# jkulhanek/tetra-nerf

Hardware: NVIDIA H100
Metric: rays/sec (4096-ray batch, 300k-tet mesh) (higher is better)
Workload: dtype f32 (trace/interp/compositing) + f16w2 tensor-core MLP (fp16 activations x fp16 hi/lo weights, f32 accumulate; per-sample density/colour within 1e-4 of the fp32 oracle, tests/test_gpu_render.py)

## Files before the change

### tetra-nerf_b200/csrc/tn_common.cuh

```cuda
#pragma once
#include <cuda_runtime.h>
#include <stdint.h>

#include <atomic>
#include <string>

#include "../../include/tetranerf_b200.h"

#define TN_EMPTY 0xFFFFFFFFu

namespace tn {

void set_error(const std::string &msg);
int fail(int code, const std::string &msg);

#define TN_CUDA(expr)                                                                                       \
    do {                                                                                                    \
        cudaError_t _e = (expr);                                                                            \
        if (_e != cudaSuccess)                                                                              \
            return tn::fail(TN_ERR_CUDA, std::string(#expr) + " failed: " + cudaGetErrorString(_e) + " (" + \
                                             __FILE__ + ":" + std::to_string(__LINE__) + ")");              \
    } while (0)

#define TN_TRY(...)                              \
    do {                                         \
        const int _rc = (__VA_ARGS__);           \
        if (_rc != TN_OK) return _rc;            \
    } while (0)

inline std::atomic<uint64_t> g_device_bytes{0};

template <typename T>
struct DevArray {
    T *p = nullptr;
    size_t cap = 0;

    DevArray() = default;
    DevArray(const DevArray &) = delete;
    DevArray &operator=(const DevArray &) = delete;
    DevArray(DevArray &&o) noexcept : p(o.p), cap(o.cap) { o.p = nullptr; o.cap = 0; }
    DevArray &operator=(DevArray &&o) noexcept {
        if (this != &o) {
            release();
            p = o.p; cap = o.cap;
            o.p = nullptr; o.cap = 0;
        }
        return *this;
    }
    ~DevArray() { release(); }

    int grow(size_t n) {
        if (n <= cap) return TN_OK;
        release();
        const size_t bytes = (n * sizeof(T) + 255) / 256 * 256;
        void *q = nullptr;
        TN_CUDA(cudaMalloc(&q, bytes));
        p = static_cast<T *>(q);
        cap = bytes / sizeof(T);
        g_device_bytes += cap * sizeof(T);
        return TN_OK;
    }

// ... 300 lines not shown
```

### tetra-nerf_b200/csrc/tn_render.cu

```cuda
#include <atomic>
#include <cmath>
#include <vector>

#include <cstddef>
#include <cstdlib>
#include <cub/cub.cuh>
#include "tn_background.cuh"
#include "tn_common.cuh"
#include "tn_composite.cuh"
#include "tn_direnc.cuh"
#include "tn_mlp.cuh"
#include "tn_mlp_bwd.cuh"
#include "tn_mlp_pack.cuh"
#include "tn_sort.cuh"

namespace tn {

int launch_trace_internal(tn_tracer *h, const float *o, const float *d, uint32_t R, uint32_t M, uint32_t *num, uint32_t *cells, float *bary,
                          float *dist, uint32_t *verts, int dense, cudaStream_t s);

struct TrainBufs {
    uint32_t *n_active;
    uint32_t *ray_list;
    float *ebins_f, *sbins_f;
    uint4 *vi_f;
    float *bary_f;
    float *out_f;
    float *dirbias, *enc;
    float *dirs;
};

constexpr uint32_t SAVED_MAGIC = 0x53564e54u;
struct SavedHeader {
    uint32_t magic, R, M, Sc, Sf, S2, det;
    uint32_t edepth;
    float bg[3];
    uint32_t pad2;
    uint64_t gen;
    uint64_t mesh_gen;
    uint32_t cull;
    uint32_t live_c, live_f;
    uint32_t pad3;
    uint32_t bgmap;
    uint32_t bg_H, bg_W, pad4;
    uint64_t bg_gen;
};

struct RenderState {
    DevArray<float> fshadow;
    uint32_t V = 0;
    DevArray<uint8_t> wimg;
    DevArray<uint8_t> wimg16;
    int mlp_prec = 2;
    DevArray<float> bias;
    DevArray<float> head;
    DevArray<float> w4dir;
    bool have_weights = false;
    uint64_t gen = 0;
    DevArray<uint32_t> num, cells, verts;
    DevArray<float> bary, dist;
    DevArray<float> ebins_c, sbins_c, bary_c, dens_c;
    DevArray<uint4> vi_c;
    DevArray<uint8_t> own;
    TrainBufs own_b{};
    SavedHeader last{};
    DevArray<uint8_t> wimg_bwd;
    DevArray<float4> dout;
    DevArray<float> gshadow, gw, g_dirbias;
    float *peer[8] = {nullptr, nullptr, nullptr, nullptr, nullptr, nullptr, nullptr, nullptr};
    uint32_t gather_world = 0, gather_rank = 0, gather_stride = 0;
    bool profile = false;
    cudaEvent_t ev[7] = {nullptr, nullptr, nullptr, nullptr, nullptr, nullptr, nullptr};
// ... 73 lines not shown
    const uint32_t v0 = blockIdx.x * 32;
    for (uint32_t c = threadIdx.y; c < 64; c += blockDim.y) {
        const uint32_t v = v0 + threadIdx.x;
        tile[c][threadIdx.x] = v < V ? in[(size_t)c * V + v] : 0.f;
    }
    __syncthreads();
    for (uint32_t r = threadIdx.y; r < 32; r += blockDim.y) {
        const uint32_t v = v0 + r;
        if (v < V) {
            out[(size_t)v * 64 + field_pos(threadIdx.x)] = tile[threadIdx.x][r];
            out[(size_t)v * 64 + field_pos(32 + threadIdx.x)] = tile[32 + threadIdx.x][r];
        }
    }
}

__global__ void k_pack_small(const float *b1, const float *b2, const float *b3, const float *w4, const float *b4, const float *wc,
                             const float *bc, const float *wd, const float *bd, float *bias, float *head, float *w4dir) {
    const int t = threadIdx.x;
    bias[t] = b1[t]; bias[128 + t] = b2[t]; bias[256 + t] = b3[t];
    head[t] = wd[t];
    head[128 + t] = wc[t]; head[256 + t] = wc[128 + t]; head[384 + t] = wc[256 + t];
    if (t == 0) { head[512] = bd[0]; head[513] = bc[0]; head[514] = bc[1]; head[515] = bc[2]; }
    for (int k = 0; k < 27; ++k) w4dir[t * 27 + k] = w4[t * 155 + k];
    w4dir[128 * 27 + t] = b4[t];
}

constexpr int SAMPLE_WARPS = 4;

struct SampleParams {
    uint32_t R, M, Sc, Sf, S2, biased;
    const uint32_t *num;
    const float2 *dist;
    const uint4 *verts;
    const float *bary;
    const float *o, *d;
    uint32_t *n_active, *ray_list;
    float *ebins_c, *sbins_c, *bary_c;
    uint4 *vi_c;
    const float *dens_c;
    float *ebins_f, *bary_f;
    uint4 *vi_f;
    float *dirbias;
    const float *w4dir;
    const float *out_f;
    float *rgb, *acc, *depth;
    uint8_t *mask;
    float far_plane, bg0, bg1, bg2;
    uint32_t train;
    const float *jit_c, *jit_f;
    float *sbins_f, *enc;
    float *peer[8];
    uint32_t gather_world, gather_rank, gather_stride;
    const uint32_t *ray_slot;
    float *edepth;
    uint32_t *dbounds;
    const uint32_t *cells;
    const float *occ;
    float occ_thr;
    const float *bgmap;
    uint32_t bg_H, bg_W;
};

#define TN_CULLED 0xFFFFFFFEu
__device__ __forceinline__ bool cell_culled(const SampleParams &p, uint32_t cell) { return cell != TN_EMPTY && __ldg(p.occ + cell) < p.occ_thr; }
__device__ __forceinline__ void cull_sample(const SampleParams &p, size_t row, uint32_t seg, uint4 &vi, float &b0, float &b1, float &b2) {
    if (vi.x == TN_EMPTY) return;
    if (cell_culled(p, __ldg(p.cells + row + seg))) {
        vi = make_uint4(TN_EMPTY, TN_EMPTY, TN_EMPTY, TN_CULLED);
        b0 = b1 = b2 = 0.f;
    }
}

__device__ __forceinline__ void store_pixel(const SampleParams &p, uint32_t ray, int lane, float r, float g, float b, float a, float depth, uint8_t mask) {
    if (lane == 0) {
        p.rgb[3 * (size_t)ray] = r; p.rgb[3 * (size_t)ray + 1] = g; p.rgb[3 * (size_t)ray + 2] = b;
        p.acc[ray] = a; p.depth[ray] = depth;
        if (p.mask != nullptr) p.mask[ray] = mask;
    }
    if ((uint32_t)lane < p.gather_world) {
        float2 *dst = reinterpret_cast<float2 *>(p.peer[lane] + 6 * ((size_t)p.gather_rank * p.gather_stride + ray));
        dst[0] = make_float2(r, g); dst[1] = make_float2(b, a); dst[2] = make_float2(depth, mask ? 1.f : 0.f);
        __threadfence_system();
    }
}

__device__ void smem_scan_max(const float *in, float *out, uint32_t n, int lane) {
    float carry = -3.0e38f;
    for (uint32_t base = 0; base < n; base += 32) {
        const uint32_t i = base + lane;
        float v = i < n ? in[i] : -3.0e38f;
#pragma unroll
        for (int o = 1; o < 32; o <<= 1) {
            const float t = __shfl_up_sync(0xffffffffu, v, o);
            if (lane >= o) v = fmaxf(v, t);
        }
        v = fmaxf(v, carry);
        if (i < n) out[i] = v;
        carry = __shfl_sync(0xffffffffu, v, 31);
    }
    __syncwarp();
}
__device__ __forceinline__ float linspace_f(float start, float end, uint32_t steps, uint32_t i) {
    const float step = (end - start) / (float)(steps - 1);
    return i < steps / 2 ? start + step * (float)i : end - step * (float)(steps - i - 1);
}

__device__ __forceinline__ uint32_t match_sample(float d, uint32_t n, const float2 *__restrict__ dist, const float *pm, size_t row,
                                                 const uint4 *__restrict__ verts, const float *__restrict__ bary, uint4 &vi, float &b0,
                                                 float &b1, float &b2) {
    vi = make_uint4(TN_EMPTY, TN_EMPTY, TN_EMPTY, TN_EMPTY);
    b0 = b1 = b2 = 0.f;
    uint32_t lo = 0, hi = n;
    while (lo < hi) {
        const uint32_t mid = (lo + hi) >> 1;
        if (pm[mid] < d) lo = mid + 1; else hi = mid;
    }
    if (lo >= n) return lo;
    const float2 h = __ldg(dist + row + lo);
    if (h.x <= d) {
        vi = __ldg(verts + row + lo);
        const float mult = __fdiv_rn(__fsub_rn(d, h.x), __fsub_rn(h.y, h.x));
        const float omm = __fsub_rn(1.0f, mult);
        const float *c = bary + 6 * (row + lo);
        b0 = __fadd_rn(__fmul_rn(omm, __ldg(c)), __fmul_rn(mult, __ldg(c + 3)));
        b1 = __fadd_rn(__fmul_rn(omm, __ldg(c + 1)), __fmul_rn(mult, __ldg(c + 4)));
        b2 = __fadd_rn(__fmul_rn(omm, __ldg(c + 2)), __fmul_rn(mult, __ldg(c + 5)));
    }
    return lo;
}

__host__ __device__ __forceinline__ size_t seg_arr(uint32_t M) { return (size_t)M + 2; }
__host__ __device__ __forceinline__ size_t coarse_floats(uint32_t M, uint32_t Sc, uint32_t biased) { return seg_arr(M) * (biased ? 2 : 1) + (size_t)Sc + 2; }
__host__ __device__ __forceinline__ size_t fine_floats(uint32_t M, uint32_t Smax) { return seg_arr(M) + 4 * ((size_t)Smax + 2); }
__host__ __device__ __forceinline__ size_t place_floats(uint32_t M, uint32_t Sc) { return 3 * seg_arr(M) + (size_t)Sc + 2; }

template <bool ORDERED, bool PLACE = false>
__global__ void __launch_bounds__(SAMPLE_WARPS * 32) k_sample_coarse(const SampleParams p) {
    extern __shared__ float sm[];
    const int warp = threadIdx.x >> 5, lane = threadIdx.x & 31;
    const uint32_t ray = blockIdx.x * SAMPLE_WARPS + warp;
    if (ray >= p.R) return;
    const uint32_t M = p.M, S = p.Sc;
    const size_t A = seg_arr(M);
    float *pm = sm + (size_t)warp * (PLACE ? place_floats(M, S) : coarse_floats(M, S, p.biased));
    float *cum = pm + A, *e = PLACE ? cum + 2 * A : cum + (p.biased ? A : 0);
    const uint32_t n = p.num[ray];
    if constexpr (ORDERED) {
        if (ray == p.R - 1 && lane == 0) *p.n_active = p.ray_slot[ray] + (n > 0 ? 1u : 0u);
    }
    if (n == 0) {
        float b0 = p.bg0, b1 = p.bg1, b2 = p.bg2;
        if (p.bgmap != nullptr) {
            bg_lookup(p.bgmap, p.bg_H, p.bg_W, p.d[3 * (size_t)ray], p.d[3 * (size_t)ray + 1], p.d[3 * (size_t)ray + 2], b0, b1, b2);
            if (!p.train) { b0 = fminf(fmaxf(b0, 0.f), 1.f); b1 = fminf(fmaxf(b1, 0.f), 1.f); b2 = fminf(fmaxf(b2, 0.f), 1.f); }
        }
        store_pixel(p, ray, lane, b0, b1, b2, 0.f, p.far_plane, 0);
        return;
    }
    uint32_t slot = 0;
    if constexpr (ORDERED) {
        slot = p.ray_slot[ray];
        if (lane == 0) { p.ray_list[slot] = ray; p.mask[ray] = 1; }
    } else {
        if (lane == 0) { slot = atomicAdd(p.n_active, 1u); p.ray_list[slot] = ray; p.mask[ray] = 1; }
        slot = __shfl_sync(0xffffffffu, slot, 0);
    }
    const size_t row = (size_t)ray * M;
    const float near = __ldg(&p.dist[row]).x, far = __ldg(&p.dist[row + n - 1]).y;
    bool placed = false;
    uint32_t nk = 0;
    uint32_t *kix = reinterpret_cast<uint32_t *>(cum + A);
    if constexpr (PLACE) {
        for (uint32_t base = 0; base < n; base += 32) {
            const uint32_t k = base + lane;
            const bool kept = k < n && !cell_culled(p, __ldg(p.cells + row + k));
            const uint32_t bal = __ballot_sync(0xffffffffu, kept);
            if (kept) kix[nk + __popc(bal & ((1u << lane) - 1u))] = k;
            nk += __popc(bal);
        }
        placed = nk > 0 && nk < n;
    }
    for (uint32_t k = lane; k < n; k += 32) {
        const float2 h = __ldg(&p.dist[row + k]);
        pm[k] = h.y;
        if (p.biased && !placed) cum[k + 1] = fmaxf(h.y - h.x, 0.f);
    }
    if (p.biased && !placed && lane == 0) cum[0] = near;
    if (placed && !p.biased) {
        __syncwarp();
        for (uint32_t i = lane; i < nk; i += 32) {
            const float2 h = __ldg(&p.dist[row + kix[i]]);
            cum[i + 1] = fmaxf(h.y - h.x, 0.f);
        }
        if (lane == 0) cum[0] = 0.f;
    }
    __syncwarp();
    smem_scan_max(pm, pm, n, lane);
    if (p.biased && !placed) {
        smem_scan_add(cum, n + 1, lane);
    }
    if (placed) {
        if (!p.biased) smem_scan_add(cum, nk + 1, lane);
        for (uint32_t j = lane; j <= S; j += 32) {
            float b = linspace_f(0.f, 1.f, S + 1, j);
            if (p.jit_c != nullptr) {
                const float lower = j == 0 ? b : (b + linspace_f(0.f, 1.f, S + 1, j - 1)) / 2.0f;
                const float upper = j == S ? b : (linspace_f(0.f, 1.f, S + 1, j + 1) + b) / 2.0f;
                b = lower + (upper - lower) * __ldg(p.jit_c + (size_t)ray * (S + 1) + j);
            }
// ... 11 lines not shown
            } else {
                const float x = b * cum[nk];
                uint32_t lo = 1, hi = nk;
                while (lo < hi) { const uint32_t mid = (lo + hi) >> 1; if (cum[mid] <= x) lo = mid + 1; else hi = mid; }
                i = lo - 1;
                off = x - cum[i];
            }
            const float2 h = __ldg(&p.dist[row + kix[i]]);
            e[j] = fminf(h.x + off, fmaxf(h.x, h.y));
        }
        __syncwarp();
        smem_scan_max(e, e, S + 1, lane);
        for (uint32_t j = lane; j <= S; j += 32) {
            p.ebins_c[(size_t)slot * (S + 1) + j] = e[j];
            p.sbins_c[(size_t)slot * (S + 1) + j] = (e[j] - near) / (far - near);
        }
    } else {
        for (uint32_t j = lane; j <= S; j += 32) {
            float b = linspace_f(0.f, 1.f, S + 1, j);
            if (p.jit_c != nullptr) {
                const float lower = j == 0 ? b : (b + linspace_f(0.f, 1.f, S + 1, j - 1)) / 2.0f;
                const float upper = j == S ? b : (linspace_f(0.f, 1.f, S + 1, j + 1) + b) / 2.0f;
                b = lower + (upper - lower) * __ldg(p.jit_c + (size_t)ray * (S + 1) + j);
            }
            float eu = b * far + (1.f - b) * near;
            float sb = b;
            if (p.biased) {
                const float uni = (eu - near) / (far - near);
                float rest = uni * (float)n;
                float iv = fminf(floorf(rest), (float)(n - 1));
                iv = fmaxf(iv, 0.f);
                rest = rest - iv;
                const uint32_t k = (uint32_t)iv;
                const float2 hk = __ldg(&p.dist[row + k]);
                const float len = fmaxf(hk.y - hk.x, 0.f);
                eu = cum[k] + len * rest;
                sb = (eu - near) / (far - near);
            }
            e[j] = eu;
            p.ebins_c[(size_t)slot * (S + 1) + j] = eu;
            p.sbins_c[(size_t)slot * (S + 1) + j] = sb;
        }
    }
    __syncwarp();
    for (uint32_t j = lane; j < S; j += 32) {
        const float dmid = (e[j + 1] + e[j]) / 2.f;
        uint4 vi; float b0, b1, b2;
        const uint32_t seg = match_sample(dmid, n, p.dist, pm, row, p.verts, p.bary, vi, b0, b1, b2);
        if (p.occ != nullptr) cull_sample(p, row, seg, vi, b0, b1, b2);
        const size_t g = (size_t)slot * S + j;
        p.vi_c[g] = vi;
        p.bary_c[3 * g] = b0; p.bary_c[3 * g + 1] = b1; p.bary_c[3 * g + 2] = b2;
    }
}

__device__ __forceinline__ void dir_bias(const SampleParams &p, uint32_t ray, uint32_t slot, int lane) {
    const float dx = p.d[3 * (size_t)ray], dy = p.d[3 * (size_t)ray + 1], dz = p.d[3 * (size_t)ray + 2];
    float enc[27];
    encode_direction(dx, dy, dz, enc);
    if (p.train) {
#pragma unroll
        for (int k = 0; k < 27; ++k) if (lane == k) p.enc[(size_t)slot * 27 + k] = enc[k];
    }
    for (uint32_t o = lane; o < 128; o += 32) {
        float acc = p.w4dir[128 * 27 + o];
#pragma unroll
        for (int k = 0; k < 27; ++k) acc = fmaf(__ldg(p.w4dir + o * 27 + k), enc[k], acc);
        p.dirbias[(size_t)slot * 128 + o] = acc;
    }
}

__global__ void __launch_bounds__(SAMPLE_WARPS * 32) k_sample_fine(const SampleParams p) {
    extern __shared__ float sm[];
    const int warp = threadIdx.x >> 5, lane = threadIdx.x & 31;
    const uint32_t slot = blockIdx.x * SAMPLE_WARPS + warp;
    if (slot >= *p.n_active) return;
    const uint32_t M = p.M, S = p.Sc, S2 = p.S2, nb = p.Sf + 1;
    const size_t A = seg_arr(M), B = (size_t)max(p.Sc, p.S2) + 2;
    float *pm = sm + (size_t)warp * fine_floats(M, max(p.Sc, p.S2));
    float *cdf = pm + A, *e = cdf + B, *x = e + B, *y = x + B;
    const uint32_t ray = p.ray_list[slot];
    const uint32_t n = p.num[ray];
    const size_t row = (size_t)ray * M;
    const float near = __ldg(&p.dist[row]).x, far = __ldg(&p.dist[row + n - 1]).y;
    for (uint32_t k = lane; k < n; k += 32) pm[k] = __ldg(&p.dist[row + k]).y;
    __syncwarp();
    smem_scan_max(pm, pm, n, lane);
    const float *eb = p.ebins_c + (size_t)slot * (S + 1);
    const float *sbc = p.sbins_c + (size_t)slot * (S + 1);
    for (uint32_t j = lane; j < S; j += 32) x[j] = (eb[j + 1] - eb[j]) * p.dens_c[(size_t)slot * S + j];
    __syncwarp();
    weights_from_density(x, y, S, lane);
    float part = 0.f;
    for (uint32_t j = lane; j < S; j += 32) { x[j] = x[j] + 0.01f; part += x[j]; }
    float wsum = warp_sum_f(part);
    const float padding = fmaxf(1e-5f - wsum, 0.f);
    wsum += padding;
    for (uint32_t j = lane; j < S; j += 32) y[j] = (x[j] + padding / (float)S) / wsum;
    __syncwarp();
    smem_scan_add(y, S, lane);
    if (lane == 0) cdf[0] = 0.f;
    for (uint32_t j = lane; j < S; j += 32) cdf[j + 1] = fminf(1.f, y[j]);
    __syncwarp();
    const float u_end = (float)(1.0 - 1.0 / (double)nb), u_off = (float)(1.0 / (2.0 * (double)nb));
    for (uint32_t i = lane; i < nb; i += 32) {
        const float u = linspace_f(0.f, u_end, nb, i) + (p.jit_f != nullptr ? __ldg(p.jit_f + (size_t)ray * nb + i) / (float)nb : u_off);
// ... 606 lines not shown
    if (r && r->gather_world && d_normals != nullptr)
        return fail(TN_ERR_ARG, "tn_render: the fused pixel gather (tn_render_set_gather) carries no normals; switch it off first");
    if (!r || !r->fshadow.p || !r->have_weights) return fail(TN_ERR_STATE, "tn_render: call tn_render_set_field and tn_render_set_weights first");
    if (!h->mesh.nodes.p) return fail(TN_ERR_STATE, "tn_render: no tetrahedra loaded");
    if (r->V != h->mesh.V) return fail(TN_ERR_ARG, "tn_render: field has a different vertex count than the mesh");
    const uint32_t M = cfg->max_ray_triangles, Sc = cfg->num_samples, Sf = cfg->num_fine_samples;
    if (Sc == 0 || Sc > 4096 || Sf > 4096) return fail(TN_ERR_ARG, "tn_render: num_samples must be in [1,4096]");
    if (tf != nullptr && Sf == 0) return fail(TN_ERR_ARG, "tn_render_train_forward: the fused training step needs num_fine_samples > 0");
    const bool det = tf != nullptr && r->det;
    if (det && (uint64_t)R * (Sc + Sf + 1) * 4 > 0x7FFFFFFFull)
        return fail(TN_ERR_ARG, "tn_render_train_forward: deterministic mode takes at most 2^29 fine samples per call (split the batch)");
    if (R == 0) return TN_OK;
    if ((uint64_t)R * (uint64_t)(Sc + Sf + 1) >= (1ull << 32)) return fail(TN_ERR_ARG, "tn_render: rays x samples must stay below 2^32 per call (split the batch)");
    const bool single = Sf == 0;
    const bool cull = r->occ != nullptr;
    if (cull && r->occ_T != h->mesh.T)
        return fail(TN_ERR_STATE, "tn_render: the occupancy was set for a mesh with another number of tetrahedra (tn_render_set_occupancy)");
    const uint32_t S2 = single ? Sc : Sc + Sf + 1;
    DeviceGuard g(h->device);
    cudaStream_t s = (cudaStream_t)stream;
    const bool place = cull && r->occ_place;
    const size_t smem_sc = SAMPLE_WARPS * sizeof(float) * (place ? place_floats(M, Sc) : coarse_floats(M, Sc, cfg->use_biased_sampler));
    const size_t smem_sf = SAMPLE_WARPS * sizeof(float) * fine_floats(M, std::max(Sc, S2));
    const size_t smem_c = SAMPLE_WARPS * sizeof(float) * 2 * ((size_t)S2 + 2);
    const size_t smem_cb = SAMPLE_WARPS * sizeof(float) * 4 * ((size_t)S2 + 2);
    if (!r->smem_optin) TN_CUDA(cudaDeviceGetAttribute(&r->smem_optin, cudaDevAttrMaxSharedMemoryPerBlockOptin, h->device));
    {
        size_t need = std::max(smem_sc, smem_c);
        const char *kern = smem_sc >= smem_c ? "k_sample_coarse" : "k_composite";
        if (!single && smem_sf > need) { need = smem_sf; kern = "k_sample_fine"; }
        if (tf != nullptr && smem_cb > need) { need = smem_cb; kern = "k_composite_bwd"; }
        if (need > (size_t)r->smem_optin)
            return fail(TN_ERR_ARG, "tn_render: num_samples + num_fine_samples = " + std::to_string(Sc + Sf) + " at max_ray_triangles = " +
                                        std::to_string(M) + " needs " + std::to_string(need) + " bytes of shared memory per block in " + kern +
                                        ", above the device's shared-memory limit of " + std::to_string(r->smem_optin) +
                                        " bytes (fewer samples or a smaller max_ray_triangles)");
    }
    TN_TRY(ensure_ws(r, R, M, Sc));
    const bool own = tf == nullptr || tf->saved == nullptr;
    const bool keep_dirs = tf != nullptr && r->bgmap != nullptr;
    if (own) TN_TRY(r->own.grow(saved_layout(R, S2, nullptr, nullptr, tf == nullptr, keep_dirs)));
    if (d_normals != nullptr) TN_TRY(r->grad_n.grow((size_t)R * S2));
    if (tf != nullptr) TN_TRY(ensure_train_ws(r, R, S2, r->V));
    r->last = SavedHeader{};
    TrainBufs b{};
    saved_layout(R, S2, own ? r->own.p : (uint8_t *)tf->saved, &b, tf == nullptr, keep_dirs);
    if (own) r->own_b = b;
    const int prec = tf != nullptr ? 3 : r->mlp_prec;
    TN_CUDA(cudaMemsetAsync(b.n_active, 0, 16, s));
    if (d_edepth != nullptr) {
        TN_CUDA(cudaMemsetAsync(b.n_active + 4, 0xff, 4, s));
        TN_CUDA(cudaMemsetAsync(b.n_active + 5, 0, 4, s));
    }
#define TN_EV(i) do { if (r->profile) cudaEventRecord(r->ev[i], s); } while (0)
    TN_EV(0);
    {
        const void *extra[2] = {r->fshadow.p, prec == 2 ? r->wimg16.p : r->wimg.p};
        const size_t extra_b[2] = {sizeof(float) * 64 * (size_t)r->V, 32768 + 3 * 65536};
        const int rc = launch_prefetch(h, extra, extra_b, 2, s);
        if (rc) return rc;
    }
    int rc = launch_trace_internal(h, d_origins, d_directions, R, M, r->num.p, r->cells.p, r->bary.p, r->dist.p, r->verts.p, 0, s);
    if (rc) return rc;
    TN_EV(1);
    SampleParams p{};
    p.R = R; p.M = M; p.Sc = Sc; p.Sf = Sf; p.S2 = S2; p.biased = cfg->use_biased_sampler;
    p.num = r->num.p; p.dist = (const float2 *)r->dist.p; p.verts = (const uint4 *)r->verts.p; p.bary = r->bary.p;
    p.o = d_origins; p.d = d_directions; p.n_active = b.n_active; p.ray_list = b.ray_list;
    p.ebins_c = r->ebins_c.p; p.sbins_c = r->sbins_c.p; p.bary_c = r->bary_c.p; p.vi_c = r->vi_c.p; p.dens_c = r->dens_c.p;
    p.ebins_f = b.ebins_f; p.bary_f = b.bary_f; p.vi_f = b.vi_f; p.dirbias = b.dirbias; p.w4dir = r->w4dir.p; p.out_f = b.out_f;
    p.rgb = d_rgb; p.acc = d_acc; p.depth = d_depth; p.mask = d_mask;
    p.far_plane = cfg->far_plane; p.bg0 = cfg->background[0]; p.bg1 = cfg->background[1]; p.bg2 = cfg->background[2];
    if (tf != nullptr) { p.train = 1; p.jit_c = tf->jit_c; p.jit_f = tf->jit_f; p.sbins_f = b.sbins_f; p.enc = b.enc; }
    p.edepth = d_edepth; p.dbounds = b.n_active + 4;
    if (cull) { p.cells = r->cells.p; p.occ = r->occ; p.occ_thr = r->occ_thr; }
    if (r->bgmap != nullptr) { p.bgmap = r->bgmap; p.bg_H = r->bg_H; p.bg_W = r->bg_W; }
    if (keep_dirs) TN_CUDA(cudaMemcpyAsync(b.dirs, d_directions, 12 * (size_t)R, cudaMemcpyDeviceToDevice, s));
    if (r->gather_world) {
        if (R > r->gather_stride) return fail(TN_ERR_ARG, "tn_render: more rays than the gathered-pixel buffers were sized for (tn_render_set_gather)");
        for (int k = 0; k < 8; ++k) p.peer[k] = r->peer[k];
        p.gather_world = r->gather_world; p.gather_rank = r->gather_rank; p.gather_stride = r->gather_stride;
    }
    auto k_coarse_sample = place ? (det ? k_sample_coarse<true, true> : k_sample_coarse<false, true>) : (det ? k_sample_coarse<true> : k_sample_coarse<false>);
    TN_CUDA(cudaFuncSetAttribute(k_coarse_sample, cudaFuncAttributeMaxDynamicSharedMemorySize, (int)smem_sc));
    if (!single) TN_CUDA(cudaFuncSetAttribute(k_sample_fine, cudaFuncAttributeMaxDynamicSharedMemorySize, (int)smem_sf));
    auto k_comp = d_edepth != nullptr ? k_composite<true> : k_composite<false>;
    TN_CUDA(cudaFuncSetAttribute(k_comp, cudaFuncAttributeMaxDynamicSharedMemorySize, (int)smem_c));
    auto launch_coarse = cull ? (prec == 2 ? launch_mlp<false, 2, true> : launch_mlp<false, 3, true>) : (prec == 2 ? launch_mlp<false, 2> : launch_mlp<false, 3>);
    auto launch_fine = cull ? (prec == 2 ? launch_mlp<true, 2, true> : launch_mlp<true, 3, true>) : (prec == 2 ? launch_mlp<true, 2> : launch_mlp<true, 3>);
    const uint32_t gridR = (R + SAMPLE_WARPS - 1) / SAMPLE_WARPS;

    if (det) {
        rc = ordered_slots(r, R, s);
        if (rc) return rc;
        p.ray_slot = r->ray_slot.p;
        h->launches += 2;
    }
    k_coarse_sample<<<gridR, SAMPLE_WARPS * 32, smem_sc, s>>>(p);
    TN_EV(2);
    MlpParams mc{};
    mc.n_active = b.n_active; mc.S = Sc; mc.vi = r->vi_c.p; mc.bary = r->bary_c.p; mc.fshadow = r->fshadow.p; mc.wimg = prec == 2 ? r->wimg16.p : r->wimg.p;
    mc.bias = r->bias.p; mc.head = r->head.p; mc.dirbias = nullptr; mc.out = r->dens_c.p;
    mc.tile_ctr = b.n_active + 1;
    int sms = 132;
    cudaDeviceGetAttribute(&sms, cudaDevAttrMultiProcessorCount, h->device);
    const uint64_t tiles_c = ((uint64_t)R * Sc + MLP_TILE - 1) / MLP_TILE, tiles_f = ((uint64_t)R * S2 + MLP_TILE - 1) / MLP_TILE;
    const uint32_t grid_c = (uint32_t)std::min<uint64_t>((tiles_c + MLP_WGS - 1) / MLP_WGS, (uint64_t)sms);
    const uint32_t grid_f = (uint32_t)std::min<uint64_t>((tiles_f + MLP_WGS - 1) / MLP_WGS, (uint64_t)sms);
    if (!single) {
        if (cull) {
            TN_TRY(compact_rows(h, r, b.n_active, Sc, R, r->vi_c.p, r->dens_c.p, 1, r->rowmap_c, b.n_active + 6, s));
            mc.rowmap = r->rowmap_c.p; mc.n_rows = b.n_active + 6;
        }
        rc = launch_coarse(mc, grid_c, s);
        if (rc) return rc;
    }
    TN_EV(3);
    if (!single) k_sample_fine<<<gridR, SAMPLE_WARPS * 32, smem_sf, s>>>(p);
    else k_dirbias_only<<<gridR, SAMPLE_WARPS * 32, 0, s>>>(p);
    TN_EV(4);
    MlpParams mf = mc;
    mf.S = S2; mf.dirbias = b.dirbias; mf.out = b.out_f;
    if (!single) { mf.vi = b.vi_f; mf.bary = b.bary_f; }
    else p.ebins_f = r->ebins_c.p;
    mf.tile_ctr = b.n_active + 2;
    if (cull) {
        TN_TRY(compact_rows(h, r, b.n_active, S2, R, mf.vi, b.out_f, 4, r->rowmap_f, b.n_active + 7, s));
        mf.rowmap = r->rowmap_f.p; mf.n_rows = b.n_active + 7;
    }
    rc = launch_fine(mf, grid_f, s);
    if (rc) return rc;
    TN_EV(5);
    k_comp<<<gridR, SAMPLE_WARPS * 32, smem_c, s>>>(p);
    TN_EV(6);
#undef TN_EV
    h->launches += 5;
    TN_CUDA(cudaGetLastError());
    if (d_edepth != nullptr) {
        k_expected_depth_finalize<<<(R + 255) / 256, 256, 0, s>>>(R, r->num.p, p.dbounds, cfg->far_plane, d_edepth);
        h->launches += 1;
        TN_CUDA(cudaGetLastError());
    }
    if (d_normals != nullptr) {
        NormalsLaunch nl{};
        nl.n_active = b.n_active; nl.ray_list = b.ray_list; nl.tile_ctr = b.n_active + 3;
        nl.S = S2; nl.R = R; nl.prec = (uint32_t)prec; nl.vi = mf.vi; nl.bary = mf.bary; nl.ebins = p.ebins_f; nl.out_f = b.out_f;
        nl.fshadow = r->fshadow.p; nl.wimg = mf.wimg; nl.bias = r->bias.p; nl.head = r->head.p; nl.xyz = h->mesh.xyz; nl.grad = r->grad_n.p;
        nl.normals = d_normals;
        rc = launch_normals(nl, sms, s);
        if (rc) return rc;
        h->launches += 2;
// ... 420 lines not shown
```

### tetra-nerf_b200/csrc/tn_trace.cu

```cuda
#include <algorithm>
#include <cstdlib>

#include "tn_common.cuh"
#include "tn_pairing.cuh"

namespace tn {

using namespace pairing;
constexpr int TRACE_WARPS = 4;

struct TraceParams {
    const float *o, *d;
    uint32_t R, M;
    uint32_t *num, *cells;
    float *bary, *dist;
    uint32_t *verts;
    const float4 *nodes;
    const LeafRec *leaves;
    const uint4 *tri;
    const uint2 *tt;
    const float *xyz;
    BvhLevels lv;
    float absmax;
    int dense;
    int *flags;
    uint32_t hcap, scap, lcap;
    uint32_t *ovf_count, *ovf_list;
    const uint32_t *ray_count, *ray_list;
    const u64 *keys_in;
};

__device__ __forceinline__ uint32_t warp_incl_scan(uint32_t v, int lane) {
#pragma unroll
    for (int o = 1; o < 32; o <<= 1) {
        const uint32_t t = __shfl_up_sync(FULL, v, o);
        if (lane >= o) v += t;
    }
    return v;
}
__device__ u64 rank_select(u64 *hits, uint32_t &nh, uint32_t keep, int lane) {
    u64 f0 = 0, f1 = 0;
    for (uint32_t k = 0; lane + 32 * k < nh; ++k) {
        const u64 key = hits[lane + 32 * k];
        uint32_t rank = 0;
        for (uint32_t j = 0; j < nh; ++j) rank += (hits[j] < key) ? 1u : 0u;
        if (rank < keep) { if (k < 64) f0 |= 1ull << k; else f1 |= 1ull << (k - 64); }
    }
    __syncwarp();
    uint32_t base = 0;
    u64 mx = 0;
    for (uint32_t k = 0; 32 * k < nh; ++k) {
        const uint32_t i = lane + 32 * k;
        const bool kp = i < nh && (((k < 64) ? (f0 >> k) : (f1 >> (k - 64))) & 1ull);
        const u64 key = kp ? hits[i] : 0ull;
        const uint32_t mask = __ballot_sync(FULL, kp);
        __syncwarp();
        if (kp) { hits[base + __popc(mask & ((1u << lane) - 1u))] = key; mx = key > mx ? key : mx; }
        base += __popc(mask);
        __syncwarp();
    }
#pragma unroll
    for (int o = 16; o > 0; o >>= 1) { const u64 t = __shfl_xor_sync(FULL, mx, o); mx = t > mx ? t : mx; }
    nh = base;
    return mx;
}

template <int MODE>
__global__ void __launch_bounds__(TRACE_WARPS * 32, 7) k_trace(const TraceParams p) {
    extern __shared__ __align__(16) unsigned char smem_raw[];
    __shared__ uint32_t s_count[TN_MAX_LEVELS], s_offset[TN_MAX_LEVELS];
    if (threadIdx.x < TN_MAX_LEVELS) { s_count[threadIdx.x] = p.lv.count[threadIdx.x]; s_offset[threadIdx.x] = p.lv.offset[threadIdx.x]; }
    __syncthreads();
    const int warp = threadIdx.x >> 5, lane = threadIdx.x & 31;
    const size_t per_warp = (size_t)p.hcap * 8 + (size_t)p.scap * 4 + (size_t)p.lcap * 4;
    unsigned char *base = smem_raw + (size_t)warp * per_warp;
    u64 *hits = reinterpret_cast<u64 *>(base);
    uint32_t *stack = reinterpret_cast<uint32_t *>(base + (size_t)p.hcap * 8);
    uint32_t *leafq = stack + p.scap;
    const uint32_t M = p.M;

    const uint32_t nwork = p.ray_list ? *p.ray_count : p.R;
    for (uint32_t wi = blockIdx.x * TRACE_WARPS + warp; wi < nwork; wi += gridDim.x * TRACE_WARPS) {
        const uint32_t entry = p.ray_list ? p.ray_list[wi] : wi;
        const uint32_t ray = entry & 0x7FFFFFFFu;
        const bool provided = p.keys_in != nullptr && (entry >> 31) != 0u;
        const float ox = p.o[3 * (size_t)ray], oy = p.o[3 * (size_t)ray + 1], oz = p.o[3 * (size_t)ray + 2];
        const float dx = p.d[3 * (size_t)ray], dy = p.d[3 * (size_t)ray + 1], dz = p.d[3 * (size_t)ray + 2];
        const RaySetup rs = ray_setup(ox, oy, oz, dx, dy, dz);
        const float ix = __fdiv_rn(1.0f, dx), iy = __fdiv_rn(1.0f, dy), iz = __fdiv_rn(1.0f, dz);
        const float pad = 4e-6f * (fmaxf(fabsf(ox), fmaxf(fabsf(oy), fabsf(oz))) + p.absmax);

        uint32_t sc = 0, lc = 0, nh = 0;
        u64 cutoff = ~0ull;
        bool overflow = false, deferred = false;
        if (provided) {
            nh = p.num[ray];
            for (uint32_t i = lane; i < nh; i += 32) hits[i] = p.keys_in[(size_t)ray * M + i];
        } else if (rs.valid) {
            if (lane == 0) stack[0] = (uint32_t)(p.lv.nlevels - 1) << 28;
            sc = 1;
        }
        __syncwarp();

        while (sc | lc) {
            if (lc >= 32 || sc == 0) {
                const uint32_t room = (p.hcap - nh) >> 2;
                const uint32_t n = min(min(lc, 32u), room);
                if (n == 0) {
                    if (p.ovf_list != nullptr) { deferred = true; break; }
                    cutoff = rank_select(hits, nh, M - 1, lane);
                    continue;
                }
                u64 k0 = 0, k1 = 0, k2 = 0, k3 = 0;
                uint32_t fl = 0;
                if (lane < n) {
                    const uint32_t pos = leafq[lc - 1 - lane];
                    const float4 *lp = reinterpret_cast<const float4 *>(p.leaves + pos);
                    const float4 v0 = __ldg(lp), v1 = __ldg(lp + 1), v2 = __ldg(lp + 2), v3 = __ldg(lp + 3);
                    const Sheared s0 = shear(rs, v0.x, v0.y, v0.z), s1 = shear(rs, v1.x, v1.y, v1.z);
                    const Sheared s2 = shear(rs, v2.x, v2.y, v2.z), s3 = shear(rs, v3.x, v3.y, v3.z);
                    const uint32_t f0 = __float_as_uint(v0.w), f1 = __float_as_uint(v1.w), f2 = __float_as_uint(v2.w), f3 = __float_as_uint(v3.w);
                    float t, u, v;
                    if ((f0 >> 31) && tri_test(s1, s2, s3, t, u, v)) { k0 = ((u64)__float_as_uint(t) << 32) | (f0 & TN_FACE_MASK); if (k0 < cutoff) fl |= 1u; }
                    if ((f1 >> 31) && tri_test(s2, s3, s0, t, u, v)) { k1 = ((u64)__float_as_uint(t) << 32) | (f1 & TN_FACE_MASK); if (k1 < cutoff) fl |= 2u; }
                    if ((f2 >> 31) && tri_test(s3, s0, s1, t, u, v)) { k2 = ((u64)__float_as_uint(t) << 32) | (f2 & TN_FACE_MASK); if (k2 < cutoff) fl |= 4u; }
                    if ((f3 >> 31) && tri_test(s0, s1, s2, t, u, v)) { k3 = ((u64)__float_as_uint(t) << 32) | (f3 & TN_FACE_MASK); if (k3 < cutoff) fl |= 8u; }
                }
                const uint32_t c = __popc(fl);
                const uint32_t incl = warp_incl_scan(c, lane);
                const uint32_t total = __shfl_sync(FULL, incl, 31);
                uint32_t w = nh + incl - c;
                if (fl & 1u) hits[w++] = k0;
                if (fl & 2u) hits[w++] = k1;
                if (fl & 4u) hits[w++] = k2;
                if (fl & 8u) hits[w++] = k3;
                nh += total;
                lc -= n;
                __syncwarp();
            } else {
                const uint32_t n = min(min(sc, 32u), (p.scap - sc) / (TN_FAN - 1u));
                if (n == 0) { if (p.ovf_list != nullptr) deferred = true; else overflow = true; break; }
                uint32_t hm = 0, cl = 1, cbase = 0;
                if (lane < n) {
                    const uint32_t e = stack[sc - 1 - lane];
                    cl = (e >> 28) - 1u;
                    cbase = (e & 0x0FFFFFFFu) << TN_FAN_LOG2;
                    const uint32_t nc = min(TN_FAN, s_count[cl] - cbase);
                    const float4 *np = p.nodes + 2 * (size_t)(s_offset[cl] + cbase);
#pragma unroll
// ... 83 lines not shown
        if (lane == 0) p.num[ray] = jc;
        __syncwarp();
    }
}

struct PrefetchArgs {
    const void *ptr[8];
    unsigned long long bytes[8];
    int n;
};
__global__ void k_l2_prefetch(const PrefetchArgs a) {
    const unsigned long long CH = 16384ull;
    unsigned long long base = 0;
    const unsigned long long tid = (unsigned long long)blockIdx.x * blockDim.x + threadIdx.x, nth = (unsigned long long)gridDim.x * blockDim.x;
    for (int i = 0; i < a.n; ++i) {
        const unsigned long long nch = (a.bytes[i] + CH - 1) / CH;
        for (unsigned long long c = (tid + nth - base % nth) % nth; c < nch; c += nth) {
            const unsigned long long off = c * CH;
            const unsigned int sz = (unsigned int)min(CH, a.bytes[i] - off) & ~15u;
            if (sz) asm volatile("cp.async.bulk.prefetch.L2.global [%0], %1;" ::"l"((const char *)a.ptr[i] + off), "r"(sz) : "memory");
        }
        base += nch;
    }
}

int launch_prefetch(tn_tracer *h, const void *const *extra, const size_t *extra_bytes, int nextra, cudaStream_t s) {
    const Mesh &m = h->mesh;
    PrefetchArgs a{};
    int n = 0;
    auto add = [&](const void *p, size_t b) { if (p && b && n < 8 && ((uintptr_t)p & 15) == 0) { a.ptr[n] = p; a.bytes[n] = b; ++n; } };
    if (m.walkable) {
        add(m.walk.p, sizeof(WalkRec) * (size_t)m.T);
        add(m.hull_leaves.p, sizeof(LeafRec) * (size_t)m.H);
        add(m.hull_nodes.p, sizeof(float4) * 2 * (size_t)(m.hull_lv.offset[m.hull_lv.nlevels - 1] + TN_FAN));
    } else {
        const uint32_t total_nodes = m.lv.offset[m.lv.nlevels - 1] + TN_FAN;
        add(m.nodes.p, sizeof(float4) * 2 * (size_t)total_nodes);
        add(m.leaves.p, sizeof(LeafRec) * (size_t)m.T);
    }
    add(m.tri.p, sizeof(uint4) * (size_t)m.F);
    add(m.tt.p, sizeof(uint2) * (size_t)m.F);
    add(m.xyz, sizeof(float) * 3 * (size_t)m.V);
    for (int i = 0; i < nextra; ++i) add(extra[i], extra_bytes[i]);
    a.n = n;
    int sms = 132;
    cudaDeviceGetAttribute(&sms, cudaDevAttrMultiProcessorCount, h->device);
    k_l2_prefetch<<<sms, 128, 0, s>>>(a);
    h->launches += 1;
    TN_CUDA(cudaGetLastError());
    return TN_OK;
}

static int launch_trace(tn_tracer *h, int mode, const float *o, const float *d, uint32_t R, uint32_t M, uint32_t *num, uint32_t *cells,
                        float *bary, float *dist, uint32_t *verts, int dense, cudaStream_t s) {
    if (!h) return fail(TN_ERR_ARG, "null tracer");
    if (M == 0 || (M & (M - 1)) != 0) return fail(TN_ERR_ARG, "max_ray_triangles must be a power of 2.");
    if (M < 2 || M > 2048) return fail(TN_ERR_ARG, "max_ray_triangles must be in [2, 2048]");
    if (!h->mesh.nodes.p) return fail(TN_ERR_STATE, "trace_rays: no tetrahedra loaded (call load_tetrahedra first)");
    if (R == 0) return TN_OK;
    DeviceGuard g(h->device);
    TraceParams p{};
    p.o = o; p.d = d; p.R = R; p.M = M; p.num = num; p.cells = cells; p.bary = bary; p.dist = dist; p.verts = verts;
    p.nodes = h->mesh.nodes.p; p.leaves = h->mesh.leaves.p; p.tri = h->mesh.tri.p; p.tt = h->mesh.tt.p;
    p.xyz = h->mesh.xyz; p.lv = h->mesh.lv; p.absmax = h->mesh.absmax; p.dense = dense; p.flags = h->d_flags.p;
    auto kern = mode == 0 ? k_trace<0> : k_trace<1>;
    int sms = 132;
    cudaDeviceGetAttribute(&sms, cudaDevAttrMultiProcessorCount, h->device);
    auto launch = [&](uint32_t nblocks_wanted) -> int {
        const size_t smem = (size_t)TRACE_WARPS * ((size_t)p.hcap * 8 + (size_t)p.scap * 4 + (size_t)p.lcap * 4);
        TN_CUDA(cudaFuncSetAttribute(kern, cudaFuncAttributeMaxDynamicSharedMemorySize, (int)smem));
        int occ = 1;
        TN_CUDA(cudaOccupancyMaxActiveBlocksPerMultiprocessor(&occ, kern, TRACE_WARPS * 32, smem));
        if (occ < 1) occ = 1;
        const uint32_t grid = std::min<uint32_t>(nblocks_wanted, (uint32_t)(sms * occ));
        kern<<<grid, TRACE_WARPS * 32, smem, s>>>(p);
        h->launches += 1;
        TN_CUDA(cudaGetLastError());
        return TN_OK;
    };
    const uint32_t want = (R + TRACE_WARPS - 1) / TRACE_WARPS;
    const bool thread_walk = R >= h->walk_min_rays;
    const bool quad_walk = !thread_walk && R >= h->walk_quad_min_rays && R <= h->walk_quad_max_rays;
    const bool solo_walk = !thread_walk && !quad_walk && R >= h->walk_solo_min_rays && R <= h->walk_solo_max_rays;
    if (mode == 0 && h->mesh.walkable && M >= 4 && (thread_walk || solo_walk || quad_walk)) {
        const size_t need = (size_t)R * M;
        TN_TRY(h->d_walk_keys.grow(need));
        TN_TRY(h->d_ovf_list.grow(R));
        uint32_t *list_count = reinterpret_cast<uint32_t *>(h->d_flags.p + 2);
        TN_CUDA(cudaMemsetAsync(list_count, 0, 2 * sizeof(uint32_t), s));
        int rc = launch_walk(h, o, d, R, M, num, cells, bary, dist, verts, h->d_walk_keys.p, h->d_ovf_list.p, list_count, thread_walk ? 0 : (quad_walk ? 2 : 1), s);
        if (rc) return rc;
        p.dense = 0;
        p.hcap = M + 128; p.scap = 4096; p.lcap = M > 512 ? M / 2 : 320;
        p.ray_count = list_count; p.ray_list = h->d_ovf_list.p; p.keys_in = h->d_walk_keys.p;
        rc = launch((uint32_t)sms);
        if (rc) return rc;
        if (dense) return launch_tail_fill(h, R, M, num, cells, bary, dist, verts, s);
        return TN_OK;
    }
    TN_TRY(h->d_ovf_list.grow(R));
    uint32_t *ovf_count = reinterpret_cast<uint32_t *>(h->d_flags.p + 2);
    TN_CUDA(cudaMemsetAsync(ovf_count, 0, sizeof(uint32_t), s));
    p.hcap = M <= 256 ? M + 128 : M; p.scap = 640; p.lcap = 320; p.ovf_count = ovf_count; p.ovf_list = h->d_ovf_list.p;
    int rc = launch(want);
    if (rc) return rc;
    p.hcap = M + 128; p.scap = 4096; p.lcap = M > 512 ? M / 2 : 320;
    p.ovf_count = nullptr; p.ovf_list = nullptr; p.ray_count = ovf_count; p.ray_list = h->d_ovf_list.p;
    return launch((uint32_t)sms);
}

int launch_trace_internal(tn_tracer *h, const float *o, const float *d, uint32_t R, uint32_t M, uint32_t *num, uint32_t *cells, float *bary,
                          float *dist, uint32_t *verts, int dense, cudaStream_t s) {
    return launch_trace(h, 0, o, d, R, M, num, cells, bary, dist, verts, dense, s);
}

}

extern "C" int tn_trace_rays(tn_tracer *h, const float *d_origins, const float *d_directions, uint32_t R, uint32_t M, uint32_t *d_num,
                             uint32_t *d_cells, float *d_bary, float *d_dist, uint32_t *d_verts, int dense, void *stream) {
    return tn::launch_trace(h, 0, d_origins, d_directions, R, M, d_num, d_cells, d_bary, d_dist, d_verts, dense, (cudaStream_t)stream);
}

extern "C" int tn_trace_rays_triangles(tn_tracer *h, const float *d_origins, const float *d_directions, uint32_t R, uint32_t M,
                                       uint32_t *d_num, uint32_t *d_faces, float *d_bary, float *d_dist, uint32_t *d_verts, void *stream) {
    return tn::launch_trace(h, 1, d_origins, d_directions, R, M, d_num, d_faces, d_bary, d_dist, d_verts, 1, (cudaStream_t)stream);
}
```

### tetra-nerf_b200/csrc/tn_walk.cu

```cuda
#include "tn_common.cuh"

namespace tn {
typedef unsigned long long u64;
#define TN_EPS 1e-6f

struct WalkParams {
    const float *o, *d;
    uint32_t R, M;
    uint32_t *num, *cells;
    float *bary, *dist;
    uint32_t *verts;
    const WalkRec *walk;
    const float4 *hull_nodes;
    const LeafRec *hull_leaves;
    const uint32_t *hull_tet;
    BvhLevels hlv;
    float absmax;
    u64 *keys;
    uint32_t *list, *list_count;
};

constexpr int WALK_THREADS = 32;
__device__ __forceinline__ uint32_t sel4u(uint32_t k, uint32_t a, uint32_t b, uint32_t c, uint32_t d) { return k == 0 ? a : (k == 1 ? b : (k == 2 ? c : d)); }

__device__ __forceinline__ void list_exact(const WalkParams &p, uint32_t ray) {
    p.list[atomicAdd(p.list_count, 1u)] = ray;
    atomicAdd(p.list_count + 1, 1u);
    p.num[ray] = 0;
}
__device__ __forceinline__ void finish_walk(const WalkParams &p, uint32_t ray, bool exact, bool generic, uint32_t nfaces, uint32_t nrec) {
    if (exact) {
        list_exact(p, ray);
    } else if (!generic) {
        p.list[atomicAdd(p.list_count, 1u)] = ray | 0x80000000u;
        p.num[ray] = nfaces;
    } else {
        p.num[ray] = nrec;
    }
}

__global__ void __launch_bounds__(WALK_THREADS) k_walk(const WalkParams p) {
    __shared__ float ssm[12][WALK_THREADS];
    const int tid = threadIdx.x;
    const uint32_t ray = blockIdx.x * blockDim.x + threadIdx.x;
    if (ray >= p.R) return;
    const float ox = p.o[3 * (size_t)ray], oy = p.o[3 * (size_t)ray + 1], oz = p.o[3 * (size_t)ray + 2];
    const float dx = p.d[3 * (size_t)ray], dy = p.d[3 * (size_t)ray + 1], dz = p.d[3 * (size_t)ray + 2];
    const RaySetup rs = ray_setup(ox, oy, oz, dx, dy, dz);
    if (!rs.valid) { p.num[ray] = 0; return; }
    const size_t row = (size_t)ray * p.M;

    u64 best = ~0ull;
    float bu = 0.f, bv = 0.f;
    uint32_t btet = TN_EMPTY, bj = 0, hullhits = 0;
    {
        const float ix = __fdiv_rn(1.0f, dx), iy = __fdiv_rn(1.0f, dy), iz = __fdiv_rn(1.0f, dz);
        const float pad = 4e-6f * (fmaxf(fabsf(ox), fmaxf(fabsf(oy), fabsf(oz))) + p.absmax);
        uint32_t stack[7 * TN_MAX_LEVELS + 8];
        int sp = 0;
        stack[sp++] = (uint32_t)(p.hlv.nlevels - 1) << 28;
        while (sp) {
            const uint32_t e = stack[--sp];
            const uint32_t cl = (e >> 28) - 1u, cbase = (e & 0x0FFFFFFFu) << TN_FAN_LOG2;
            const uint32_t nc = min(TN_FAN, p.hlv.count[cl] - cbase);
            for (uint32_t c = 0; c < nc; ++c) {
                const float4 *np = p.hull_nodes + 2 * (size_t)(p.hlv.offset[cl] + cbase + c);
                if (!slab(__ldg(np), __ldg(np + 1), ox, oy, oz, ix, iy, iz, pad)) continue;
                if (cl != 0) { stack[sp++] = (cl << 28) | (cbase + c); continue; }
                const float4 *lp = reinterpret_cast<const float4 *>(p.hull_leaves + cbase + c);
                const float4 v0 = __ldg(lp), v1 = __ldg(lp + 1), v2 = __ldg(lp + 2), v3 = __ldg(lp + 3);
                const uint32_t f[4] = {__float_as_uint(v0.w), __float_as_uint(v1.w), __float_as_uint(v2.w), __float_as_uint(v3.w)};
                if (!((f[0] | f[1] | f[2] | f[3]) & TN_FACE_HULL)) continue;
                const Sheared s[4] = {shear(rs, v0.x, v0.y, v0.z), shear(rs, v1.x, v1.y, v1.z), shear(rs, v2.x, v2.y, v2.z), shear(rs, v3.x, v3.y, v3.z)};
#pragma unroll
                for (int j = 0; j < 4; ++j) {
                    if (!(f[j] & TN_FACE_HULL)) continue;
                    float t, u, v;
                    if (tri_test(s[(j + 1) & 3], s[(j + 2) & 3], s[(j + 3) & 3], t, u, v)) {
                        const u64 k = ((u64)__float_as_uint(t) << 32) | (f[j] & TN_FACE_MASK);
                        hullhits++;
                        if (k < best) { best = k; bu = u; bv = v; btet = p.hull_tet[cbase + c]; bj = (uint32_t)j; }
                    }
                }
            }
        }
    }
    if (btet == TN_EMPTY) { p.num[ray] = 0; return; }
    if (hullhits != 2) { list_exact(p, ray); return; }
// ... 307 lines not shown
```

Before: 4.246 million.

## Overlap coarse sampling with trace fix-up pass via programmatic dependent launch

The walk kernel now marks rays that still need the BVH fix-up trace pass with a high-bit flag in num. The coarse sampling kernel is launched with programmatic stream serialization, and the trace kernel triggers dependents early. Rays already finished by the walk are sampled immediately, and only flagged rays wait on griddepcontrol.wait before reading their results. The direction copy is also moved ahead of tracing. This is meant to hide the tail of the fix-up trace pass, but it relies on the flag protocol and on memory visibility being correct for rays processed early.

```diff
diff --git a/tetra-nerf_b200/csrc/tn_common.cuh b/tetra-nerf_b200/csrc/tn_common.cuh
--- a/tetra-nerf_b200/csrc/tn_common.cuh
+++ b/tetra-nerf_b200/csrc/tn_common.cuh
@@ -8,6 +8,7 @@
 #include "../../include/tetranerf_b200.h"
 
 #define TN_EMPTY 0xFFFFFFFFu
+#define TN_LISTED 0x80000000u
 
 namespace tn {
 
diff --git a/tetra-nerf_b200/csrc/tn_launch.cuh b/tetra-nerf_b200/csrc/tn_launch.cuh
--- /dev/null
+++ b/tetra-nerf_b200/csrc/tn_launch.cuh
@@ -0,0 +1,22 @@
+#pragma once
+#include <cuda_runtime.h>
+
+#include <utility>
+
+namespace tn {
+
+__device__ __forceinline__ void pdl_wait() { asm volatile("griddepcontrol.wait;" ::: "memory"); }
+__device__ __forceinline__ void pdl_trigger() { asm volatile("griddepcontrol.launch_dependents;" ::: "memory"); }
+
+template <typename... KArgs, typename... Args>
+inline cudaError_t launch_pdl(void (*kern)(KArgs...), dim3 grid, dim3 block, size_t smem, cudaStream_t s, Args &&...args) {
+    cudaLaunchAttribute attr[1];
+    attr[0].id = cudaLaunchAttributeProgrammaticStreamSerialization;
+    attr[0].val.programmaticStreamSerializationAllowed = 1;
+    cudaLaunchConfig_t cfg{};
+    cfg.gridDim = grid; cfg.blockDim = block; cfg.dynamicSmemBytes = smem; cfg.stream = s;
+    cfg.attrs = attr; cfg.numAttrs = 1;
+    return cudaLaunchKernelEx(&cfg, kern, std::forward<Args>(args)...);
+}
+
+}
diff --git a/tetra-nerf_b200/csrc/tn_render.cu b/tetra-nerf_b200/csrc/tn_render.cu
--- a/tetra-nerf_b200/csrc/tn_render.cu
+++ b/tetra-nerf_b200/csrc/tn_render.cu
@@ -9,6 +9,7 @@
 #include "tn_common.cuh"
 #include "tn_composite.cuh"
 #include "tn_direnc.cuh"
+#include "tn_launch.cuh"
 #include "tn_mlp.cuh"
 #include "tn_mlp_bwd.cuh"
 #include "tn_mlp_pack.cuh"
@@ -17,7 +18,7 @@
 namespace tn {
 
 int launch_trace_internal(tn_tracer *h, const float *o, const float *d, uint32_t R, uint32_t M, uint32_t *num, uint32_t *cells, float *bary,
-                          float *dist, uint32_t *verts, int dense, cudaStream_t s);
+                          float *dist, uint32_t *verts, int dense, cudaStream_t s, bool *walked);
 
 struct TrainBufs {
     uint32_t *n_active;
@@ -197,6 +198,7 @@
     float *peer[8];
     uint32_t gather_world, gather_rank, gather_stride;
     const uint32_t *ray_slot;
+    uint32_t overlap;
     float *edepth;
     uint32_t *dbounds;
     const uint32_t *cells;
@@ -284,12 +286,14 @@
     extern __shared__ float sm[];
     const int warp = threadIdx.x >> 5, lane = threadIdx.x & 31;
     const uint32_t ray = blockIdx.x * SAMPLE_WARPS + warp;
-    if (ray >= p.R) return;
+    if (ray >= p.R) { pdl_wait(); return; }
     const uint32_t M = p.M, S = p.Sc;
     const size_t A = seg_arr(M);
     float *pm = sm + (size_t)warp * (PLACE ? place_floats(M, S) : coarse_floats(M, S, p.biased));
     float *cum = pm + A, *e = PLACE ? cum + 2 * A : cum + (p.biased ? A : 0);
-    const uint32_t n = p.num[ray];
+    uint32_t n = __ldcg(p.num + ray);
+    const bool early = p.overlap && !(n & TN_LISTED);
+    if (!early) { pdl_wait(); n = __ldcg(p.num + ray); }
     if constexpr (ORDERED) {
         if (ray == p.R - 1 && lane == 0) *p.n_active = p.ray_slot[ray] + (n > 0 ? 1u : 0u);
     }
@@ -300,6 +304,7 @@
             if (!p.train) { b0 = fminf(fmaxf(b0, 0.f), 1.f); b1 = fminf(fmaxf(b1, 0.f), 1.f); b2 = fminf(fmaxf(b2, 0.f), 1.f); }
         }
         store_pixel(p, ray, lane, b0, b1, b2, 0.f, p.far_plane, 0);
+        if (early) pdl_wait();
         return;
     }
     uint32_t slot = 0;
@@ -417,6 +422,7 @@
         p.vi_c[g] = vi;
         p.bary_c[3 * g] = b0; p.bary_c[3 * g + 1] = b1; p.bary_c[3 * g + 2] = b2;
     }
+    if (early) pdl_wait();
 }
 
 __device__ __forceinline__ void dir_bias(const SampleParams &p, uint32_t ray, uint32_t slot, int lane) {
@@ -1129,6 +1135,7 @@
         TN_CUDA(cudaMemsetAsync(b.n_active + 4, 0xff, 4, s));
         TN_CUDA(cudaMemsetAsync(b.n_active + 5, 0, 4, s));
     }
+    if (keep_dirs) TN_CUDA(cudaMemcpyAsync(b.dirs, d_directions, 12 * (size_t)R, cudaMemcpyDeviceToDevice, s));
 #define TN_EV(i) do { if (r->profile) cudaEventRecord(r->ev[i], s); } while (0)
     TN_EV(0);
     {
@@ -1137,7 +1144,8 @@
         const int rc = launch_prefetch(h, extra, extra_b, 2, s);
         if (rc) return rc;
     }
-    int rc = launch_trace_internal(h, d_origins, d_directions, R, M, r->num.p, r->cells.p, r->bary.p, r->dist.p, r->verts.p, 0, s);
+    bool walked = false;
+    int rc = launch_trace_internal(h, d_origins, d_directions, R, M, r->num.p, r->cells.p, r->bary.p, r->dist.p, r->verts.p, 0, s, &walked);
     if (rc) return rc;
     TN_EV(1);
     SampleParams p{};
@@ -1152,7 +1160,6 @@
     p.edepth = d_edepth; p.dbounds = b.n_active + 4;
     if (cull) { p.cells = r->cells.p; p.occ = r->occ; p.occ_thr = r->occ_thr; }
     if (r->bgmap != nullptr) { p.bgmap = r->bgmap; p.bg_H = r->bg_H; p.bg_W = r->bg_W; }
-    if (keep_dirs) TN_CUDA(cudaMemcpyAsync(b.dirs, d_directions, 12 * (size_t)R, cudaMemcpyDeviceToDevice, s));
     if (r->gather_world) {
         if (R > r->gather_stride) return fail(TN_ERR_ARG, "tn_render: more rays than the gathered-pixel buffers were sized for (tn_render_set_gather)");
         for (int k = 0; k < 8; ++k) p.peer[k] = r->peer[k];
@@ -1173,7 +1180,9 @@
         p.ray_slot = r->ray_slot.p;
         h->launches += 2;
     }
-    k_coarse_sample<<<gridR, SAMPLE_WARPS * 32, smem_sc, s>>>(p);
+    p.overlap = walked && !det && M >= 32;
+    if (p.overlap) TN_CUDA(launch_pdl(k_coarse_sample, gridR, SAMPLE_WARPS * 32, smem_sc, s, p));
+    else k_coarse_sample<<<gridR, SAMPLE_WARPS * 32, smem_sc, s>>>(p);
     TN_EV(2);
     MlpParams mc{};
     mc.n_active = b.n_active; mc.S = Sc; mc.vi = r->vi_c.p; mc.bary = r->bary_c.p; mc.fshadow = r->fshadow.p; mc.wimg = prec == 2 ? r->wimg16.p : r->wimg.p;
diff --git a/tetra-nerf_b200/csrc/tn_trace.cu b/tetra-nerf_b200/csrc/tn_trace.cu
--- a/tetra-nerf_b200/csrc/tn_trace.cu
+++ b/tetra-nerf_b200/csrc/tn_trace.cu
@@ -2,6 +2,7 @@
 #include <cstdlib>
 
 #include "tn_common.cuh"
+#include "tn_launch.cuh"
 #include "tn_pairing.cuh"
 
 namespace tn {
@@ -78,6 +79,7 @@
     uint32_t *stack = reinterpret_cast<uint32_t *>(base + (size_t)p.hcap * 8);
     uint32_t *leafq = stack + p.scap;
     const uint32_t M = p.M;
+    pdl_trigger();
 
     const uint32_t nwork = p.ray_list ? *p.ray_count : p.R;
     for (uint32_t wi = blockIdx.x * TRACE_WARPS + warp; wi < nwork; wi += gridDim.x * TRACE_WARPS) {
@@ -94,7 +96,7 @@
         u64 cutoff = ~0ull;
         bool overflow = false, deferred = false;
         if (provided) {
-            nh = p.num[ray];
+            nh = p.num[ray] & ~TN_LISTED;
             for (uint32_t i = lane; i < nh; i += 32) hits[i] = p.keys_in[(size_t)ray * M + i];
         } else if (rs.valid) {
             if (lane == 0) stack[0] = (uint32_t)(p.lv.nlevels - 1) << 28;
@@ -284,7 +286,8 @@
 }
 
 static int launch_trace(tn_tracer *h, int mode, const float *o, const float *d, uint32_t R, uint32_t M, uint32_t *num, uint32_t *cells,
-                        float *bary, float *dist, uint32_t *verts, int dense, cudaStream_t s) {
+                        float *bary, float *dist, uint32_t *verts, int dense, cudaStream_t s, bool *walked = nullptr) {
+    if (walked) *walked = false;
     if (!h) return fail(TN_ERR_ARG, "null tracer");
     if (M == 0 || (M & (M - 1)) != 0) return fail(TN_ERR_ARG, "max_ray_triangles must be a power of 2.");
     if (M < 2 || M > 2048) return fail(TN_ERR_ARG, "max_ray_triangles must be in [2, 2048]");
@@ -327,6 +330,7 @@
         p.ray_count = list_count; p.ray_list = h->d_ovf_list.p; p.keys_in = h->d_walk_keys.p;
         rc = launch((uint32_t)sms);
         if (rc) return rc;
+        if (walked) *walked = !dense;
         if (dense) return launch_tail_fill(h, R, M, num, cells, bary, dist, verts, s);
         return TN_OK;
     }
@@ -342,8 +346,8 @@
 }
 
 int launch_trace_internal(tn_tracer *h, const float *o, const float *d, uint32_t R, uint32_t M, uint32_t *num, uint32_t *cells, float *bary,
-                          float *dist, uint32_t *verts, int dense, cudaStream_t s) {
-    return launch_trace(h, 0, o, d, R, M, num, cells, bary, dist, verts, dense, s);
+                          float *dist, uint32_t *verts, int dense, cudaStream_t s, bool *walked) {
+    return launch_trace(h, 0, o, d, R, M, num, cells, bary, dist, verts, dense, s, walked);
 }
 
 }
diff --git a/tetra-nerf_b200/csrc/tn_walk.cu b/tetra-nerf_b200/csrc/tn_walk.cu
--- a/tetra-nerf_b200/csrc/tn_walk.cu
+++ b/tetra-nerf_b200/csrc/tn_walk.cu
@@ -26,14 +26,14 @@
 __device__ __forceinline__ void list_exact(const WalkParams &p, uint32_t ray) {
     p.list[atomicAdd(p.list_count, 1u)] = ray;
     atomicAdd(p.list_count + 1, 1u);
-    p.num[ray] = 0;
+    p.num[ray] = TN_LISTED;
 }
 __device__ __forceinline__ void finish_walk(const WalkParams &p, uint32_t ray, bool exact, bool generic, uint32_t nfaces, uint32_t nrec) {
     if (exact) {
         list_exact(p, ray);
     } else if (!generic) {
         p.list[atomicAdd(p.list_count, 1u)] = ray | 0x80000000u;
-        p.num[ray] = nfaces;
+        p.num[ray] = TN_LISTED | nfaces;
     } else {
         p.num[ray] = nrec;
     }
```

Result: no change. 4.329 million (median of 6 runs) (+1.9%).
